# Ruyi-Zha/endosurf

Hardware: AMD Instinct MI355X
Metric: training rays/sec (1024 rays x 64 samples) (higher is better)
Workload: dtype f32

## Files before the change

### endosurf_amd/_lib.py

```python
from __future__ import annotations

import ctypes as C
import os

HERE = os.path.dirname(os.path.abspath(__file__))
LIB_PATH = os.path.join(HERE, "lib", "libendosurf_hip.so")

_c_float_p = C.c_void_p


class es_points(C.Structure):
    _fields_ = [("x", C.c_void_p), ("t", C.c_void_p), ("dirs", C.c_void_p), ("rays", C.c_void_p), ("z", C.c_void_p),
                ("mode", C.c_int), ("t_scalar", C.c_int), ("n_per_ray", C.c_int), ("ldz", C.c_int), ("M", C.c_int), ("M_split", C.c_int)]


class es_composite_args(C.Structure):
    _fields_ = ([(n, C.c_void_p) for n in ("rays", "z")] + [("ldz", C.c_int)]
                + [(n, C.c_void_p) for n in ("sdf", "g_o", "rgb", "variance")]
                + [("N", C.c_int), ("S", C.c_int), ("sample_dist", C.c_float), ("cos_anneal", C.c_float)]
                + [(n, C.c_void_p) for n in ("color", "depth", "weights", "cdf", "weight_max", "eik_acc", "wmax_idx",
                                             "g_color", "g_depth", "g_weights", "g_cdf", "g_wmax", "g_gradients_o", "g_eik",
                                             "eik_den", "d_sdf", "d_go", "d_rgb", "d_invs_acc", "ray_part", "cos_anneal_dev",
                                             "go_copy", "g_aux_sdf", "g_aux_go")] + [("n_aux", C.c_int)])

# ... 42 lines not shown
    "es_secant_points": (_I, [_P, _P, _I, _P, _P, _P]),
    "es_secant_update": (_I, [_P, _I, _F, _P, _P, _P]),
    "es_march_finish": (_I, [_P, _P, _I, _P, _P]),
    "es_point_workspace_floats": (C.c_int64, [_I, _I]),
    "es_point_workspace_offset": (C.c_int64, [_I, _I, _I]),
    "es_point_forward": (_I, [C.POINTER(es_points), _P, _P, _P, _I, _I, _P]),
    "es_point_forward_rows": (_I, [C.POINTER(es_points), _P, _P, _P, _I, _I, _I, _I, _P]),
    "es_eod_points": (_I, [_P, _P, _P, _I, _P, _P, _P, _P]),
    "es_sn_points": (_I, [_P, _P, _P, _P, _F, _I, _P, _P, _P, _P]),
    "es_eod_loss": (_I, [_P, _P, _P, _P, _P, _I, _P, _P, _P]),
    "es_eod_loss_backward": (_I, [_P, _P, _P, _P, _P, _P, _P, _I, _P, _P, _P]),
    "es_sn_loss": (_I, [_P, _P, _I, _P, _P]),
    "es_sn_loss_backward": (_I, [_P, _P, _P, _P, _I, _P, _P]),
    "es_copy2": (_I, [_P, _P, C.c_longlong, _P, _P, C.c_longlong, _P]),
    "es_color_forward": (_I, [C.POINTER(es_points), _P, _P, _P, _P]),
    "es_point_vjp": (_I, [C.POINTER(es_points), _P, _P, _P, _I, _P]),
    "es_point_backward_stages": (_I, [C.POINTER(es_points), _P, _P, _P, _I, _I, _P, _P, _P, _P, _P, _I, _P]),
    "es_weightnorm_backward_layers": (_I, [_P, _P, _P, _I, _I, _P]),
    "es_point_forward_x3": (_I, [C.POINTER(es_points), _P, _P, _P, _P, _I, _I, _P]),
    "es_gemm_atb": (_I, [_P, _P, _I, _P, _I, _P, _P]),
    "es_point_backward_x3": (_I, [C.POINTER(es_points), _P, _P, _P, _P, _I, _I, _P, _P, _P, _P, _P, _P]),
    "es_point_backward": (_I, [C.POINTER(es_points), _P, _P, _P, _I, _I, _P, _P, _P, _P, _P]),
    "es_wgrad_scratch_floats": (C.c_int64, []),
    "es_point_backward_det": (_I, [C.POINTER(es_points), _P, _P, _P, _I, _I, _P, _P, _P, _P, _P, _P]),
    "es_train_loss": (_I, [C.POINTER(es_loss_args), _P]),
    "es_query_sdf_rays": (_I, [C.POINTER(es_points), _P, _P, _P, _I, _P, _I, _P]),
    "es_march_progress": (_I, [_P, _I, _I, _I, C.c_float, _P, _P]),
    "es_variance_terms": (_I, [_P, _P, _P, _P, _P]),
    "es_sample_scratch_floats": (C.c_int64, [_I, _I, _I, _I]),
    "es_sample_z": (_I, [_P, _P, _I, _I, _I, _I, _I, _P, _P, _I, _P, _P, _P]),
    "es_march_scratch_floats": (C.c_int64, [_I, _I]),
    "es_ray_marching": (_I, [_P, _I, _I, _I, C.c_float, _I, _P, _P, _I, _P, _P, _P]),
    "es_render_scratch_floats": (C.c_int64, [_I, _I]),
    "es_render_forward": (_I, [C.POINTER(es_render_args), _P, _P, _P]),
    "es_render_backward": (_I, [C.POINTER(es_render_args), _P, _P, _P, _P]),
    "es_train_aux_points": (_I, [_P, _P, _P, _P, _P, C.c_float, _I, _P, _P, _P, _P]),
    "es_adam_step": (_I, [_P, _P, _P, _P, C.c_longlong, C.c_float, C.c_float, C.c_float, C.c_float, C.c_float, C.c_float, _P, C.c_longlong, _P]),
    "es_train_schedule": (_I, [_P, C.c_double, C.c_double, C.c_double, C.c_double, C.c_double, C.c_double, C.c_float, C.c_double, _P, _P]),
    "es_adam_step_dev": (_I, [_P, _P, _P, _P, C.c_longlong, C.c_float, C.c_float, C.c_float, _P, _P, C.c_longlong, _P]),
    "es_zero": (_I, [_P, C.c_longlong, _P]),
    "es_uniform": (_I, [_P, C.c_longlong, C.c_ulonglong, C.c_ulonglong, _P, _P]),
    "es_scale": (_I, [_P, _P, C.c_longlong, _P, _P]),
    "es_render_finish": (_I, [_P, _P, _P, _I, _P, _P, _P, _P, _P]),
    "es_iso_scratch_bytes": (C.c_int64, [_I, _I, _I]),
    "es_iso_count": (_I, [_P, _I, _I, _I, C.c_double, _P, _P, _P]),
    "es_iso_emit": (_I, [_P, _I, _I, _I, C.c_double, _P, C.c_longlong, C.c_longlong, _P, _P, _P, _P]),
# ... 105 lines not shown
```

### endosurf_amd/csrc/api.hip

```cpp
#include "arch.h"
#include "chain_common.h"
#include "host.h"
#include "launch.h"
#include "workspace.h"

namespace es {
static inline PointSrc to_src(const es_points* p) { PointSrc s; static_cast<es_points&>(s) = *p; return s; }
static inline int check_src(const es_points* p) {
    ES_REQUIRE(p != nullptr, "es_points is null");
    ES_REQUIRE(p->M >= 0, "negative point count");
    if (p->M == 0) return ST_OK;
    if (p->mode == 0) {
        ES_REQUIRE(p->x && p->t, "mode 0 needs x and t");
    } else {
        ES_REQUIRE(p->mode == 1 || p->mode == 2, "unknown point-source mode");
        ES_REQUIRE(p->rays && p->z && p->n_per_ray > 0 && p->ldz >= p->n_per_ray, "modes 1/2 need rays, z, n_per_ray <= ldz");
        if (p->mode == 2) ES_REQUIRE(p->M_split >= 0 && p->M_split <= p->M && (p->M_split == p->M || (p->x && p->t)), "mode 2 needs M_split <= M and x, t");
    }
    return ST_OK;
}
static inline int check_points(const es_points* p, bool weights, bool rows) {
    if (int e = check_src(p)) return e;
    ES_REQUIRE(weights && (rows || p->M == 0), "null buffer");
    return ST_OK;
// ... 246 lines not shown
int es_point_backward_x3(const es_points* pts, const float* packed, const void* packed_x3, const float* weff, float* ws, int flags, int m_color,
                         const float* d_sdf, const float* d_go, const float* d_rgb, float* dweff, float* wg_scratch, void* stream) {
    if (int e = check_point_call(pts, packed && packed_x3 && weff && dweff, ws && d_sdf && d_go, flags, m_color, true, d_rgb)) return e;
    flags |= ES_PF_X3_CHAIN | ES_PF_X3;
    return run_backward(pts, packed, packed_x3, weff, ws, flags, m_color, d_sdf, d_go, d_rgb, dweff, wg_scratch, 15, stream);
}
int es_point_backward_det(const es_points* pts, const float* packed, const float* weff, float* ws, int flags, int m_color,
                          const float* d_sdf, const float* d_go, const float* d_rgb, float* dweff, float* wg_scratch, void* stream) {
    if (int e = check_point_call(pts, packed && weff && dweff, ws && d_sdf && d_go, flags, m_color, true, d_rgb)) return e;
    return run_backward(pts, packed, nullptr, weff, ws, flags, m_color, d_sdf, d_go, d_rgb, dweff, wg_scratch, 15, stream);
}
int es_point_backward(const es_points* pts, const float* packed, const float* weff, float* ws, int flags, int m_color,
                      const float* d_sdf, const float* d_go, const float* d_rgb, float* dweff, void* stream) {
    return es_point_backward_det(pts, packed, weff, ws, flags, m_color, d_sdf, d_go, d_rgb, dweff, nullptr, stream);
}
int es_point_backward_stages(const es_points* pts, const float* packed, const float* weff, float* ws, int flags, int m_color,
                             const float* d_sdf, const float* d_go, const float* d_rgb, float* dweff, float* wg_scratch, int stages, void* stream) {
    if (int e = check_point_call(pts, packed && weff && dweff, ws && d_sdf && d_go, flags, m_color, true, d_rgb)) return e;
    ES_REQUIRE(!(flags & ES_PF_X3_CHAIN), "the staged backward is the fp32 family's (a workspace of es_point_forward)");
    ES_REQUIRE(stages > 0 && stages < 16, "stages: ES_BWD_CHAINS | ES_BWD_WGRAD_DEFORM | ES_BWD_WGRAD_SDF | ES_BWD_WGRAD_COLOR");
    return run_backward(pts, packed, nullptr, weff, ws, flags, m_color, d_sdf, d_go, d_rgb, dweff, wg_scratch, stages, stream);
}
int64_t es_wgrad_scratch_floats(void) { return (int64_t)wgrad_det_floats(); }
int es_gemm_atb(const float* X, const float* dA, int M, float* out, int split_precision, float* wg_scratch, void* stream) {
    ES_REQUIRE(X && dA && out && M > 0 && M % 64 == 0, "es_gemm_atb: X [M][256], dA [M][256], out [256][256], M a multiple of 64");
    return gemm_atb(X, dA, M, out, split_precision, wg_scratch, (hipStream_t)stream);
}

int es_train_loss(const es_loss_args* a, void* stream) {
    ES_REQUIRE(a && a->eik, "es_train_loss inputs");
    ES_REQUIRE(a->N == 0 || (a->color_map && a->depth_map && a->aux_sdf && a->aux_go && a->rays && a->eod_pts && a->color_gt && a->depth_gt &&
                             a->mask && a->cmask && a->valid_sn), "es_train_loss inputs");
    ES_REQUIRE(a->den_out || (a->terms && a->g_eik && (a->N == 0 || (a->g_color && a->g_depth && a->g_aux_sdf && a->g_aux_go))),
               "es_train_loss outputs");
    ES_REQUIRE(!a->den_global || a->world >= 1.f, "es_train_loss: den_global needs the world size");
    return train_loss(*reinterpret_cast<const LossArgs*>(a), (hipStream_t)stream);
}

int es_zero(void* p, long long nbytes, void* stream) {
    ES_REQUIRE((p || nbytes == 0) && nbytes >= 0, "es_zero arguments");
    return zero(p, nbytes, (hipStream_t)stream);
}
int es_uniform(float* out, long long n, unsigned long long seed, unsigned long long subsequence, const double* subsequence_dev, void* stream) {
    ES_REQUIRE((out || n == 0) && n >= 0, "es_uniform arguments");
    return uniform(out, n, seed, subsequence, subsequence_dev, (hipStream_t)stream);
}
// ... 38 lines not shown
```

### endosurf_amd/csrc/host.h

```cpp
#pragma once
#include <hip/hip_runtime.h>

#include <cstddef>
#include <type_traits>

#include "../../include/endosurf_hip.h"

namespace es {

struct PointSrc; struct WsLayout; struct FwdArgs; struct BwdArgs;

struct CompositeArgs : ::es_composite_args {};
struct LossArgs : ::es_loss_args {};
static_assert(sizeof(CompositeArgs) == sizeof(es_composite_args) && std::is_standard_layout<CompositeArgs>::value, "es::CompositeArgs is es_composite_args");
static_assert(sizeof(LossArgs) == sizeof(es_loss_args) && std::is_standard_layout<LossArgs>::value, "es::LossArgs is es_loss_args");
inline const CompositeArgs& as_comp(const es_composite_args* a) { return *reinterpret_cast<const CompositeArgs*>(a); }

int init_tables();
int weightnorm_pack(const float* params, float* weff, float* packed, int use_deform, hipStream_t st);
int weightnorm_backward(const float* params, const float* dweff, float* dparams, int use_deform, hipStream_t st);
int weightnorm_backward_layers(const float* params, const float* dweff, float* dparams, int first_layer, int n_layers, hipStream_t st);

int query_sdf(const PointSrc& src, const float* packed, const float* weff, float* sdf_out, int use_deform, hipStream_t st,
              int ld_out = 0, const int* ray_done = nullptr, int tile_points = 0);
// ... 3 lines not shown
int query_sdf_x3(const PointSrc& src, const void* packed_x3, const float* weff, float* sdf_out, int use_deform, hipStream_t st, int ld_out, const int* ray_done);

int point_forward(const PointSrc& src, const float* packed, const float* weff, float* ws, int flags, int m_color, hipStream_t st,
                  const void* packed_x3 = nullptr);
int point_forward_rows(const PointSrc& src, const float* packed, const float* weff, float* ws, int flags, int m_color, int row0, int nrows, hipStream_t st);
int point_vjp(const PointSrc& src, const float* packed, const float* weff, float* ws, int flags, hipStream_t st);
int color_forward(const PointSrc& src, const float* packed, const float* weff, float* ws, hipStream_t st);
int point_backward_chains(const PointSrc& src, const float* packed, const float* weff, float* ws, int flags, int m_color,
                          const float* d_sdf, const float* d_go, const float* d_rgb, hipStream_t st, const void* packed_x3 = nullptr);

int deform_jvp_x3r(const PointSrc& src, const void* packed_r, const float* weff, float* ws, const WsLayout& L, bool save, hipStream_t st);
int deform_vjp_x3r(const PointSrc& src, const void* packed_r, const float* weff, float* ws, const WsLayout& L, bool save, hipStream_t st, int m_rows = 0);
int deform_jvp_x3r_with_tail(const FwdArgs& fa, const void* packed_r, int m_main, hipStream_t st);
int sdf_fwd_x3r(const PointSrc& src, const void* packed_r, const float* weff, float* ws, const WsLayout& L, bool deform, bool color, hipStream_t st);
int color_fwd_x3r(const PointSrc& src, const void* packed_r, const float* weff, float* ws, const WsLayout& L, bool deform, int Mcp, bool save, hipStream_t st);

int deform_tan_x3r(const PointSrc& src, const void* packed_r, const float* weff, float* ws, const WsLayout& L, const float* d_go, hipStream_t st, int m_rows = 0);
int deform_bwd_x3r_with_tail(const BwdArgs& ba, const void* packed_r, int m_main, hipStream_t st);
int color_bwd_x3r(const PointSrc& src, const void* packed_r, const float* weff, float* ws, const WsLayout& L, bool deform, int m_color, const float* d_rgb, hipStream_t st);
int deform_bwd_x3r(const void* packed_r, const float* weff, float* ws, const WsLayout& L, int M, int m_color, hipStream_t st);

int point_wgrad(int M, float* ws, int flags, int m_color, const float* d_sdf, float* dweff, float* det, hipStream_t st, int net_mask = 7);
size_t wgrad_det_floats();
int gemm_atb(const float* X, const float* dA, int M, float* out, int x3, float* det, hipStream_t st);

int ray_setup(const float* rays, const float* u, int N, int n, float sample_dist, int lin_mode, float* z, int ldz, float* near_out, float* far_out, hipStream_t st);
int upsample_step(const float* rays, const float* z_in, int ld_in, const float* sdf_in, int ld_sdf, int N, int n, int n_imp,
                  float inv_s, float* z_new, float* z_out, int ld_out, int* src_idx, hipStream_t st);
int merge_sdf(const float* sdf_in, int ld_in, const float* sdf_new, int n_imp, const int* src_idx, int ld_out, int N, int n, float* sdf_out, hipStream_t st);
int mid_z(const float* z, int ldz, int N, int S, float sample_dist, float* mid, hipStream_t st);
int composite(const CompositeArgs& a, int backward, hipStream_t st);
int variance_terms(const float* variance, const float* d_invs_acc, float* s_val, float* d_var, hipStream_t st);
int march_progress(const float* sdf, int N, int n, int n_valid, float tau, int* done, hipStream_t st);
int march_find(const float* sdf, const float* dprop, int N, int n, float tau, float* state, int* flags, float* d_pred, hipStream_t st);
int secant_points(const float* rays, const float* d_pred, int N, float* x, float* t, hipStream_t st);
int secant_update(const float* sdf_mid, int N, float tau, float* state, float* d_pred, hipStream_t st);
int march_finish(const float* d_pred, const int* flags, int N, float* d_out, hipStream_t st);
int train_aux_points(const float* rays, const float* depth_gt, const float* mask, const float* d_i, const float* u, float rad, int N, float* x, float* t, unsigned char* valid, hipStream_t st);

int eod_points(const float* rays, const float* depth_gt, const float* mask, int N, float* x, float* t, float* inside, hipStream_t st);
int sn_points(const float* rays, const float* mask, const float* d_i, const float* u, float rad, int N, float* x, float* t, unsigned char* valid, hipStream_t st);
int eod_loss(const float* rays, const float* pts, const float* mask, const float* sdf, const float* go, int N, float* out, float* inside, hipStream_t st);
int eod_loss_bwd(const float* rays, const float* inside, const float* sdf, const float* go, const float* out, const float* g_sdf_err,
                 const float* g_ang_err, int N, float* d_sdf, float* d_go, hipStream_t st);
int sn_loss(const float* g, const unsigned char* valid, int N, float* out, hipStream_t st);
int sn_loss_bwd(const float* g, const unsigned char* valid, const float* out, const float* g_loss, int N, float* d_g, hipStream_t st);
// ... 14 lines not shown
```

### endosurf_amd/csrc/wgrad.hip

```cpp
#include <hip/hip_runtime.h>

#include <type_traits>
#include <utility>

#include "arch.h"
#include "chain_common.h"
#include "host.h"
#include "launch.h"
#include "tabs.h"
#include "timing.h"
#include "workspace.h"

namespace es {

constexpr int WG_MAX_PROBS = 20;

struct WgProb {
    const float* X; const float* dA; float* out; float* bias_out;
    int ldx, lda, ldo, M, K, N, bias_stride, task_begin;
    int x_frag, a_frag;
    int round;
};
struct WgSmall {
    const float* X; const float* dA; float* out; float* bias_out;
    int ldx, lda, ldo, M, K, N, bias_stride, x_frag, round;
};
constexpr int WG_MAX_SMALL = 4;
constexpr int WG_MAX_TASKS = 512;
struct WgArgs {
    WgProb p[WG_MAX_PROBS];
    WgSmall s[WG_MAX_SMALL];
    int nprob, total_tasks, MC, nsmall;
    int KW;
    float* det;
};
constexpr size_t WG_DET_TILE = (size_t)256 * 128;
constexpr size_t WG_DET_BIAS_OFF = (size_t)WG_MAX_TASKS * WG_DET_TILE;
constexpr size_t WG_DET_SMALL_OFF = WG_DET_BIAS_OFF + (size_t)WG_MAX_TASKS * 256;
constexpr size_t WG_DET_FLOATS = WG_DET_SMALL_OFF + (size_t)WG_MAX_SMALL * WG_MAX_TASKS * 5 * 256;

__host__ __device__ inline void wg_decode(int local, int kblk, int nchunk, int& kb, int& mc) {
    if (kblk == 2) {
        const int grp = local / 16, j = local % 16;
        const int full = (nchunk / 8) * 8;
        if (grp * 8 < full) { mc = grp * 8 + (j & 7); kb = j >> 3; }
        else { const int rem = local - 2 * full; kb = rem & 1; mc = full + (rem >> 1); }
    } else { kb = local % kblk; mc = local / kblk; }
}
__host__ __device__ inline int wg_encode(int kb, int mc, int kblk, int nchunk) {
    if (kblk == 2) {
        const int full = (nchunk / 8) * 8;
        return mc < full ? (mc / 8) * 16 + (mc & 7) + 8 * kb : 2 * full + (((mc - full) << 1) | kb);
    }
    return mc * kblk + kb;
}

constexpr int WG_THREADS = 512;
constexpr int WG_R = 16;
constexpr int WG_KW = 128;
constexpr int WG_LDS_FLOATS = 2 * WG_R * (256 + WG_KW);

template <bool AF, bool XF, bool DET>
__device__ __forceinline__ void wgrad_task(const WgProb& P, int kb, int m0, int m1, float* lds, float* det_tile, float* det_bias) {
    constexpr int KW = WG_KW;
    const int tid = threadIdx.x, lane = tid & 63;
    const int w = __builtin_amdgcn_readfirstlane(tid >> 6);
    const int nb = w & 3, kh = w >> 2;
    const int lo = lane & 31, hi = lane >> 5;
    auto Apan = [&](int buf) { return lds + buf * (WG_R * 256); };
    auto Bpan = [&](int buf) { return lds + 2 * WG_R * 256 + buf * (WG_R * KW); };
    const int kcol0 = kb * KW;

    typedef float v4f_t __attribute__((ext_vector_type(4)));
    f32x16 acc[2][2];
    acc_zero(acc);
    const bool do_bias = P.bias_out != nullptr && kb == 0;
    v4f_t bsum = {0.f, 0.f, 0.f, 0.f};

    typedef float v4f __attribute__((ext_vector_type(4)));
    const v4f vzero = {0.f, 0.f, 0.f, 0.f};
    const int fa1 = tid + WG_THREADS;
    const unsigned offA0 = (unsigned)(tid >> 6) * (unsigned)P.lda + 4u * (tid & 63);
    const int colB = kcol0 + 4 * (tid % (KW / 4));
    const unsigned offB = (unsigned)(tid / (KW / 4)) * (unsigned)P.ldx + (unsigned)colB;
    const bool okB = XF || colB < P.ldx;
    const int fqq = (tid >> 6) & 1, fni = (tid >> 7) & 1, fw = tid >> 8;
    const unsigned foffA0 = (unsigned)(((fw * 16 + fni * 4 + fqq) * 64 + lane) * 4);
    const unsigned foffB = (unsigned)((((2 * kb + fw) * 16 + fni * 4 + fqq) * 64 + lane) * 4);
    const int flrow = 8 * fqq + 4 * hi;
    const int flcolA = 64 * fw + 32 * fni + lo, flcolB = 64 * fw + 32 * fni + lo;
    const unsigned boffA0 = 4u * (AF ? foffA0 : offA0), boffB = 4u * (XF ? foffB : offB);
    const size_t dA1 = AF ? (size_t)2 * 16 * 64 * 4 * 4 : (size_t)8 * P.lda * 4;
    auto stage_ptr = [&](const float* base, int ld, bool frag, int m) {
        return frag ? base + (size_t)(m >> 6) * (64 * 256) + (size_t)((8 * ((m >> 5) & 1) + 2 * ((m >> 4) & 1)) * 256) : base + (size_t)m * ld;
    };
#define WG_GLOAD(S, m)                                                                                \
    {                                                                                                 \
        const char* pa = reinterpret_cast<const char*>(stage_ptr(P.dA, P.lda, AF, m));                \
        unsigned oa0 = boffA0, ob = boffB;                                                            \
        asm volatile("" : "+v"(oa0), "+v"(ob));       \
        S##a0 = *reinterpret_cast<const v4f*>(pa + oa0);                                              \
        S##a1 = *reinterpret_cast<const v4f*>(pa + dA1 + oa0);       \
        const char* px = reinterpret_cast<const char*>(stage_ptr(P.X, P.ldx, XF, m));                 \
        S##b0 = okB ? *reinterpret_cast<const v4f*>(px + ob) : vzero;                                 \
    }
#define WG_SSTORE(S, buf)                                                                             \
    {                                                                                                 \
        if constexpr (AF) {                                                                           \
            float* la = Apan(buf) + flrow * 256 + flcolA;                                             \
            la[0] = S##a0[0]; la[256] = S##a0[1]; la[512] = S##a0[2]; la[768] = S##a0[3];             \
            la[128] = S##a1[0]; la[128 + 256] = S##a1[1]; la[128 + 512] = S##a1[2]; la[128 + 768] = S##a1[3]; \
            bsum[0] += S##a0[0] + S##a0[1] + S##a0[2] + S##a0[3];                                     \
            bsum[1] += S##a1[0] + S##a1[1] + S##a1[2] + S##a1[3];                                     \
        } else {                                                                                      \
            *reinterpret_cast<v4f*>(Apan(buf) + 4 * tid) = S##a0;                                     \
            *reinterpret_cast<v4f*>(Apan(buf) + 4 * fa1) = S##a1;                                     \
            bsum += S##a0 + S##a1;                                                                    \
        }                                                                                             \
        if constexpr (XF) {                                                                           \
            float* lb = Bpan(buf) + flrow * KW + flcolB;                                              \
            lb[0] = S##b0[0]; lb[KW] = S##b0[1]; lb[2 * KW] = S##b0[2]; lb[3 * KW] = S##b0[3];        \
        } else {                                                                                      \
            *reinterpret_cast<v4f*>(Bpan(buf) + 4 * tid) = S##b0;                                     \
        }                                                                                             \
    }
    auto compute = [&](int buf) {
        const float* A = Apan(buf) + nb * 64 + 2 * lo;
        const float* B = Bpan(buf) + kh * 64 + 2 * lo;
#pragma unroll
        for (int s = 0; s < WG_R / 2; ++s) {
            const float2 av = *reinterpret_cast<const float2*>(A + (2 * s + hi) * 256);
            const float2 bv = *reinterpret_cast<const float2*>(B + (2 * s + hi) * KW);
            acc[0][0] = __builtin_amdgcn_mfma_f32_32x32x2f32(av.x, bv.x, acc[0][0], 0, 0, 0);
            acc[0][1] = __builtin_amdgcn_mfma_f32_32x32x2f32(av.x, bv.y, acc[0][1], 0, 0, 0);
            acc[1][0] = __builtin_amdgcn_mfma_f32_32x32x2f32(av.y, bv.x, acc[1][0], 0, 0, 0);
            acc[1][1] = __builtin_amdgcn_mfma_f32_32x32x2f32(av.y, bv.y, acc[1][1], 0, 0, 0);
        }
    };

    const int nst = (m1 - m0) / WG_R;
    v4f p0a0, p0a1, p0b0, p1a0, p1a1, p1b0;
    WG_GLOAD(p0, m0);
    WG_GLOAD(p1, m0 + WG_R);
    WG_SSTORE(p0, 0);
    __syncthreads();
#pragma unroll 1
    for (int st = 0; st < nst; st += 2) {
        if (st + 2 < nst) WG_GLOAD(p0, m0 + WG_R * (st + 2));
        compute(0);
        WG_SSTORE(p1, 1);
        __syncthreads();
        if (st + 3 < nst) WG_GLOAD(p1, m0 + WG_R * (st + 3));
        compute(1);
        if (st + 2 < nst) WG_SSTORE(p0, 0);
        __syncthreads();
    }
#undef WG_GLOAD
#undef WG_SSTORE
    int tid_e = threadIdx.x;
    asm volatile("" : "+v"(tid_e));
    const int lane_e = tid_e & 63, lo_e = lane_e & 31, hi_e = lane_e >> 5;
#pragma unroll
    for (int t = 0; t < 2; ++t)
#pragma unroll
        for (int tp = 0; tp < 2; ++tp) {
            const int k = kcol0 + kh * 64 + 2 * lo_e + tp;
#pragma unroll
            for (int r = 0; r < 16; ++r) {
                const int n = nb * 64 + 2 * ((r & 3) + 8 * (r >> 2) + 4 * hi_e) + t;
                if constexpr (DET) det_tile[n * WG_KW + (k - kcol0)] = acc[t][tp][r];
                else if (n < P.N && k < P.K) atomicAdd(P.out + (size_t)n * P.ldo + k, acc[t][tp][r]);
            }
        }
    if (do_bias) {
        if (!AF && ((tid_e >> 6) & (P.bias_stride - 1)) != 0) bsum = v4f{0.f, 0.f, 0.f, 0.f};
        __syncthreads();
        if constexpr (AF) {
            const int fqq_e = (tid_e >> 6) & 1, col_e = 64 * (tid_e >> 8) + 32 * ((tid_e >> 7) & 1) + lo_e;
            lds[(fqq_e * 2 + hi_e) * 256 + col_e] = bsum[0];
            lds[(fqq_e * 2 + hi_e) * 256 + col_e + 128] = bsum[1];
        } else {
            *reinterpret_cast<v4f*>(lds + 4 * tid_e) = bsum;
        }
        __syncthreads();
        if (tid_e < 256) {
            float s = 0.f;
#pragma unroll
            for (int r = 0; r < (AF ? 4 : 8); ++r) s += lds[r * 256 + tid_e];
            if constexpr (DET) det_bias[tid_e] = s;
            else if (tid_e < P.N) atomicAdd(P.bias_out + tid_e, s);
        }
    }
}

constexpr int WS_ROWS = 16;
template <bool DET, int NH = 2>
// ... 57 lines not shown
    __syncthreads();
    float* red = lds;
    if (NH == 2 && half) {
#pragma unroll
        for (int n = 0; n < 4; ++n) red[n * 256 + k] = acc[n];
        red[1024 + k] = bsum;
    }
    if (NH == 2) __syncthreads();
    if (!half) {
        if constexpr (NH == 2) {
#pragma unroll
            for (int n = 0; n < 4; ++n) acc[n] += red[n * 256 + k];
            bsum += red[1024 + k];
        }
        if constexpr (DET) {
            for (int n = 0; n < 4; ++n) det_slot[n * 256 + k] = acc[n];
            det_slot[4 * 256 + k] = bsum;
        } else {
            for (int n = 0; n < P.N; ++n) atomicAdd(P.out + (size_t)n * P.ldo + k, acc[n]);
            if (P.bias_out && k < P.N) atomicAdd(P.bias_out + k, bsum);
        }
    }
    __syncthreads();
}

template <int NET, bool DET>
__global__ __launch_bounds__(WG_THREADS, 4) void k_wgrad(WgArgs a) {
    extern __shared__ __attribute__((aligned(16))) float wlds[];
    const int task = blockIdx.x;
    auto small_slot = [&](int i) { return DET ? a.det + WG_DET_SMALL_OFF + ((size_t)i * WG_MAX_TASKS + task) * (5 * 256) : nullptr; };
    const bool small_first = task < a.total_tasks / 2;
    if (small_first)
#pragma unroll 1
        for (int i = 0; i < a.nsmall; ++i) wgrad_small_task<DET>(a.s[i], task, a.total_tasks, wlds, small_slot(i));
    int pi = 0;
#pragma unroll 1
    for (int i = 1; i < a.nprob; ++i)
        if (task >= a.p[i].task_begin) pi = i;
    const WgProb& P = a.p[pi];
    const int local = task - P.task_begin;
    const int kblk = (P.K + WG_KW - 1) / WG_KW;
    int kb, mc;
    wg_decode(local, kblk, (P.M + a.MC - 1) / a.MC, kb, mc);
    const int m0 = mc * a.MC, m1 = min(m0 + a.MC, P.M);
    float* dt = DET ? a.det + (size_t)task * WG_DET_TILE : nullptr;
    float* db = DET ? a.det + WG_DET_BIAS_OFF + (size_t)task * 256 : nullptr;
    if constexpr (NET == 1) {
        if (P.a_frag) {
            if (P.x_frag) wgrad_task<true, true, DET>(P, kb, m0, m1, wlds, dt, db);
            else wgrad_task<true, false, DET>(P, kb, m0, m1, wlds, dt, db);
        } else {
            if (P.x_frag) wgrad_task<false, true, DET>(P, kb, m0, m1, wlds, dt, db);
            else wgrad_task<false, false, DET>(P, kb, m0, m1, wlds, dt, db);
        }
    } else {
        wgrad_task<false, false, DET>(P, kb, m0, m1, wlds, dt, db);
    }
    if (!small_first) {
        __syncthreads();
#pragma unroll 1
        for (int i = 0; i < a.nsmall; ++i) wgrad_small_task<DET>(a.s[i], task, a.total_tasks, wlds, small_slot(i));
    }
}


typedef unsigned wx_u32x4 __attribute__((ext_vector_type(4)));
typedef __bf16 wx_bf16x8 __attribute__((ext_vector_type(8)));
constexpr int WX_THREADS = 256;
constexpr int WX_R = 16;
constexpr int WX_KW = 256;
constexpr int WX_PLANE = 2 * 256 * 16;
constexpr int WX_BUF = 6 * WX_PLANE;
constexpr int WX_NBUF = 3;
constexpr int WX_LDS_BYTES = WX_NBUF * WX_BUF;
static_assert(WX_LDS_BYTES >= WG_LDS_FLOATS * 4, "the small-layer slices reuse the buffer as float scratch");

__device__ __forceinline__ unsigned wx_cvt_pk(float lo, float hi) {
    unsigned r;
    asm("v_cvt_pk_bf16_f32 %0, %1, %2" : "=v"(r) : "v"(lo), "v"(hi));
// ... 209 lines not shown
    if constexpr (NET == 1) {
        if (P.a_frag) {
            if (P.x_frag) wgrad_task_x3<true, true, DET>(P, m0, m1, wxlds, dt, db);
            else wgrad_task_x3<true, false, DET>(P, m0, m1, wxlds, dt, db);
        } else {
            if (P.x_frag) wgrad_task_x3<false, true, DET>(P, m0, m1, wxlds, dt, db);
            else wgrad_task_x3<false, false, DET>(P, m0, m1, wxlds, dt, db);
        }
    } else {
        wgrad_task_x3<false, false, DET>(P, m0, m1, wxlds, dt, db);
    }
    if (!small_first) {
#pragma unroll 1
        for (int i = 0; i < a.nsmall; ++i) wgrad_small_task<DET, 1>(a.s[i], task, a.total_tasks, wlds, small_slot(i));
    }
}

__global__ __launch_bounds__(256) void k_wgrad_reduce(WgArgs a, int round) {
    const int pi = blockIdx.y;
    const int tid0 = blockIdx.x * 256 + threadIdx.x, stride = gridDim.x * 256;
    if (pi < a.nprob) {
        const WgProb& P = a.p[pi];
        if (P.round != round) return;
        const int kblk = (P.K + a.KW - 1) / a.KW, nchunk = (P.M + a.MC - 1) / a.MC;
        const size_t tile = (size_t)256 * a.KW;
        for (int e = tid0; e < P.N * P.K; e += stride) {
            const int n = e / P.K, k = e % P.K, kb = k / a.KW, kk = k % a.KW;
            float s = 0.f;
            for (int mc = 0; mc < nchunk; ++mc)
                s += a.det[(size_t)(P.task_begin + wg_encode(kb, mc, kblk, nchunk)) * tile + n * a.KW + kk];
            P.out[(size_t)n * P.ldo + k] += s;
        }
        if (P.bias_out)
            for (int n = tid0; n < P.N; n += stride) {
                float s = 0.f;
                for (int mc = 0; mc < nchunk; ++mc)
                    s += a.det[WG_DET_BIAS_OFF + (size_t)(P.task_begin + wg_encode(0, mc, kblk, nchunk)) * 256 + n];
                P.bias_out[n] += s;
            }
    } else {
        const int i = pi - a.nprob;
        const WgSmall& P = a.s[i];
        if (P.round != round) return;
        const float* base = a.det + WG_DET_SMALL_OFF + (size_t)i * WG_MAX_TASKS * (5 * 256);
        for (int e = tid0; e < P.N * 256; e += stride) {
            const int n = e >> 8, k = e & 255;
            float s = 0.f;
            for (int t = 0; t < a.total_tasks; ++t) s += base[(size_t)t * (5 * 256) + n * 256 + k];
            P.out[(size_t)n * P.ldo + k] += s;
        }
        if (P.bias_out)
            for (int n = tid0; n < P.N; n += stride) {
                float s = 0.f;
                for (int t = 0; t < a.total_tasks; ++t) s += base[(size_t)t * (5 * 256) + 4 * 256 + n];
                P.bias_out[n] += s;
            }
    }
}

static int wg_kblk(const WgProb& p, int kw) { return (p.K + kw - 1) / kw; }

static int launch_group(WgProb* probs, int nprob, WgSmall* small, int nsmall, int kid_timer, long long rows, float* det, bool x3, hipStream_t st) {
    const int kid = kid_timer == KID_WGRAD_D_X3 ? KID_WGRAD_D : (kid_timer == KID_WGRAD_S_X3 ? KID_WGRAD_S : (kid_timer == KID_WGRAD_C_X3 ? KID_WGRAD_C : kid_timer));
    static DeviceOnce attr_done;
    if (attr_done.first()) {
        if (int e = allow_big_lds(k_wgrad<0, false>, WG_LDS_FLOATS * 4)) return e;
        if (int e = allow_big_lds(k_wgrad<1, false>, WG_LDS_FLOATS * 4)) return e;
        if (int e = allow_big_lds(k_wgrad<2, false>, WG_LDS_FLOATS * 4)) return e;
        if (int e = allow_big_lds(k_wgrad<0, true>, WG_LDS_FLOATS * 4)) return e;
        if (int e = allow_big_lds(k_wgrad<1, true>, WG_LDS_FLOATS * 4)) return e;
        if (int e = allow_big_lds(k_wgrad<2, true>, WG_LDS_FLOATS * 4)) return e;
        if (int e = allow_big_lds(k_wgrad_x3<0, false>, WX_LDS_BYTES)) return e;
        if (int e = allow_big_lds(k_wgrad_x3<1, false>, WX_LDS_BYTES)) return e;
        if (int e = allow_big_lds(k_wgrad_x3<2, false>, WX_LDS_BYTES)) return e;
        if (int e = allow_big_lds(k_wgrad_x3<0, true>, WX_LDS_BYTES)) return e;
        if (int e = allow_big_lds(k_wgrad_x3<1, true>, WX_LDS_BYTES)) return e;
        if (int e = allow_big_lds(k_wgrad_x3<2, true>, WX_LDS_BYTES)) return e;
        attr_done.done();
    }
    if (nprob == 0) return ST_OK;
    ES_REQUIRE(nprob <= WG_MAX_PROBS, "too many weight-gradient problems in one group");
    const int KW = x3 ? WX_KW : WG_KW;
    auto count = [&](int mc) {
        long long t = 0;
        for (int i = 0; i < nprob; ++i) t += (long long)wg_kblk(probs[i], KW) * ((probs[i].M + mc - 1) / mc);
        return t;
    };
    ES_REQUIRE(nsmall <= WG_MAX_SMALL, "too many small weight-gradient problems in one group");
    int MC = 128;
    const int slots = x3 ? WG_MAX_TASKS / 2 : WG_MAX_TASKS;
    while (MC < 65536 && count(MC) > slots) MC += 64;
    ES_REQUIRE(count(MC) <= slots, "weight-gradient group does not fit one round of workgroup slots");
    WgArgs a;
    a.det = det;
    int total = 0, max_round = 0;
    for (int i = 0; i < nprob; ++i) {
        ES_REQUIRE(probs[i].lda == 256 && probs[i].M % 64 == 0, "weight-gradient operands must be [64k][256] adjoints");
        ES_REQUIRE((probs[i].bias_stride & (probs[i].bias_stride - 1)) == 0, "bias stride must be a power of two");
        ES_REQUIRE(!probs[i].a_frag || probs[i].bias_stride == 1 || !probs[i].bias_out, "fragment-ordered adjoints: bias over every row");
        ES_REQUIRE(!probs[i].x_frag || (probs[i].ldx == 256 && probs[i].K == 256), "fragment-ordered inputs are [64 x 256] tiles");
        ES_REQUIRE(kid == KID_WGRAD_S || !(probs[i].x_frag || probs[i].a_frag), "fragment-ordered operands: SDF launch only");
        probs[i].task_begin = total;
        total += wg_kblk(probs[i], KW) * ((probs[i].M + MC - 1) / MC);
        probs[i].round = 0;
        for (int j = 0; j < i; ++j)
            if (probs[j].out == probs[i].out && probs[j].round >= probs[i].round) probs[i].round = probs[j].round + 1;
        max_round = probs[i].round > max_round ? probs[i].round : max_round;
        a.p[i] = probs[i];
    }
    a.nprob = nprob; a.total_tasks = total; a.MC = MC; a.nsmall = nsmall; a.KW = KW;
    for (int i = 0; i < nsmall; ++i) {
        ES_REQUIRE(small[i].K == 256 && small[i].N <= 4, "small weight-gradient problems are [<=4 x 256]");
        small[i].round = 0;
        for (int j = 0; j < i; ++j)
            if (small[j].out == small[i].out && small[j].round >= small[i].round) small[i].round = small[j].round + 1;
        max_round = small[i].round > max_round ? small[i].round : max_round;
        a.s[i] = small[i];
    }
    const dim3 grid(total);
    ScopedTimer tm(kid_timer, rows, st);
    if (x3) {
        auto reduce = [&]() {
            for (int r = 0; det && r <= max_round; ++r)
                hipLaunchKernelGGL(k_wgrad_reduce, dim3(32, nprob + nsmall), dim3(256), 0, st, a, r);
        };
        if (det) {
// ... 114 lines not shown
```

### include/endosurf_hip.h

```cpp
#ifndef ENDOSURF_HIP_H
#define ENDOSURF_HIP_H

#include <stddef.h>
#include <stdint.h>

#ifdef __cplusplus
extern "C" {
#endif

#define ES_ABI_VERSION 14

int es_abi_version(void);
const char* es_last_error(void);
int es_init(void);

int64_t es_param_floats(void);
int es_param_layout(int net, int layer, int64_t* bias_off, int64_t* g_off, int64_t* v_off, int* out_dim, int* in_dim);
int64_t es_param_variance_off(void);
int64_t es_weff_floats(void);
int es_weff_layout(int net, int layer, int64_t* w_off, int64_t* b_off);
int64_t es_packed_floats(void);

int es_weightnorm_pack(const float* params, float* weff, float* packed, int use_deform, void* stream);
int es_weightnorm_backward(const float* params, const float* dweff, float* dparams, int use_deform, void* stream);
// ... 87 lines not shown
int es_point_forward_rows(const es_points* pts, const float* packed, const float* weff, float* ws, int flags, int m_color, int row0, int nrows,
                          void* stream);
int es_point_vjp(const es_points* pts, const float* packed, const float* weff, float* ws, int flags, void* stream);
int es_color_forward(const es_points* pts, const float* packed, const float* weff, float* ws, void* stream);
int es_point_forward_x3(const es_points* pts, const float* packed, const void* packed_x3, const float* weff, float* ws, int flags, int m_color,
                        void* stream);
int es_gemm_atb(const float* X, const float* dA, int M, float* out, int split_precision, float* wg_scratch, void* stream);
int es_point_backward_x3(const es_points* pts, const float* packed, const void* packed_x3, const float* weff, float* ws, int flags, int m_color,
                         const float* d_sdf, const float* d_go, const float* d_rgb, float* dweff, float* wg_scratch, void* stream);
int es_point_backward(const es_points* pts, const float* packed, const float* weff, float* ws, int flags, int m_color,
                      const float* d_sdf, const float* d_go, const float* d_rgb, float* dweff, void* stream);

#define ES_BWD_CHAINS 1
#define ES_BWD_WGRAD_DEFORM 2
#define ES_BWD_WGRAD_SDF 4
#define ES_BWD_WGRAD_COLOR 8
int es_point_backward_stages(const es_points* pts, const float* packed, const float* weff, float* ws, int flags, int m_color,
                             const float* d_sdf, const float* d_go, const float* d_rgb, float* dweff, float* wg_scratch, int stages, void* stream);

int64_t es_wgrad_scratch_floats(void);
int es_point_backward_det(const es_points* pts, const float* packed, const float* weff, float* ws, int flags, int m_color,
                          const float* d_sdf, const float* d_go, const float* d_rgb, float* dweff, float* wg_scratch, void* stream);

int es_timing_enable(int on);
int es_timing_drain(int capacity, int* kid, long long* rows, float* ms, int* n_out);
const char* es_kernel_name(int kid);

typedef struct es_loss_args {
    const float* color_map; const float* depth_map; const float* eik; const float* aux_sdf; const float* aux_go;
    const float* rays; const float* eod_pts; const float* color_gt; const float* depth_gt; const float* mask; const float* cmask;
    const unsigned char* valid_sn;
    int N;
    float w_color, w_depth, w_sdf, w_angle, w_eik, w_sn;
    float* terms; float* g_color; float* g_depth; float* g_eik; float* g_aux_sdf; float* g_aux_go;
    float* den_out; const float* den_global; float world;
    float* total_out;
} es_loss_args;
int es_train_loss(const es_loss_args* a, void* stream);

int es_train_aux_points(const float* rays, const float* depth_gt, const float* mask, const float* d_i, const float* u, float rad, int N,
                        float* x, float* t, unsigned char* valid, void* stream);

int es_eod_points(const float* rays, const float* depth_gt, const float* mask, int N, float* x, float* t, float* inside, void* stream);
int es_sn_points(const float* rays, const float* mask, const float* d_i, const float* u, float rad, int N, float* x, float* t,
                 unsigned char* valid, void* stream);
int es_eod_loss(const float* rays, const float* pts, const float* mask, const float* sdf, const float* g_o, int N, float* out, float* inside,
// ... 102 lines not shown
```

Before: 72960.

## Specialize weight-gradient tasks by live column width and balance chunk rows per class

Adds width classes for weight-gradient k-blocks that are only partly live (at most 64 or at most 96 columns). For these, the dead half-tile skips its MFMA work or uses a single-column MFMA path, and dead B loads are replaced with zeros. A new planner gives each problem its own chunk row count, weighted by per-class cost, so narrow problems take longer M chunks and the tasks in one launch round are balanced. The cost is more template instantiations and a heuristic cost table that may not match the hardware.

```diff
diff --git a/endosurf_amd/_lib.py b/endosurf_amd/_lib.py
--- a/endosurf_amd/_lib.py
+++ b/endosurf_amd/_lib.py
@@ -88,6 +88,8 @@
     "es_point_backward_x3": (_I, [C.POINTER(es_points), _P, _P, _P, _P, _I, _I, _P, _P, _P, _P, _P, _P]),
     "es_point_backward": (_I, [C.POINTER(es_points), _P, _P, _P, _I, _I, _P, _P, _P, _P, _P]),
     "es_wgrad_scratch_floats": (C.c_int64, []),
+    "es_wgrad_plan": (_I, [_P, _P, _I, _I, _P, _P]),
+    "es_wgrad_width_cost": (C.c_double, [_I]),
     "es_point_backward_det": (_I, [C.POINTER(es_points), _P, _P, _P, _I, _I, _P, _P, _P, _P, _P, _P]),
     "es_train_loss": (_I, [C.POINTER(es_loss_args), _P]),
     "es_query_sdf_rays": (_I, [C.POINTER(es_points), _P, _P, _P, _I, _P, _I, _P]),
diff --git a/endosurf_amd/csrc/api.hip b/endosurf_amd/csrc/api.hip
--- a/endosurf_amd/csrc/api.hip
+++ b/endosurf_amd/csrc/api.hip
@@ -292,6 +292,10 @@
     return run_backward(pts, packed, nullptr, weff, ws, flags, m_color, d_sdf, d_go, d_rgb, dweff, wg_scratch, stages, stream);
 }
 int64_t es_wgrad_scratch_floats(void) { return (int64_t)wgrad_det_floats(); }
+int es_wgrad_plan(const int* rows, const int* cols, int nprob, int slots, int* chunk_rows, int* chunks) {
+    return wgrad_plan(rows, cols, nprob, slots, chunk_rows, chunks);
+}
+double es_wgrad_width_cost(int cols) { return wgrad_width_cost(cols); }
 int es_gemm_atb(const float* X, const float* dA, int M, float* out, int split_precision, float* wg_scratch, void* stream) {
     ES_REQUIRE(X && dA && out && M > 0 && M % 64 == 0, "es_gemm_atb: X [M][256], dA [M][256], out [256][256], M a multiple of 64");
     return gemm_atb(X, dA, M, out, split_precision, wg_scratch, (hipStream_t)stream);
diff --git a/endosurf_amd/csrc/host.h b/endosurf_amd/csrc/host.h
--- a/endosurf_amd/csrc/host.h
+++ b/endosurf_amd/csrc/host.h
@@ -49,6 +49,8 @@
 
 int point_wgrad(int M, float* ws, int flags, int m_color, const float* d_sdf, float* dweff, float* det, hipStream_t st, int net_mask = 7);
 size_t wgrad_det_floats();
+int wgrad_plan(const int* rows, const int* cols, int nprob, int slots, int* chunk_rows, int* chunks);
+double wgrad_width_cost(int cols);
 int gemm_atb(const float* X, const float* dA, int M, float* out, int x3, float* det, hipStream_t st);
 
 int ray_setup(const float* rays, const float* u, int N, int n, float sample_dist, int lin_mode, float* z, int ldz, float* near_out, float* far_out, hipStream_t st);
diff --git a/endosurf_amd/csrc/wgrad.hip b/endosurf_amd/csrc/wgrad.hip
--- a/endosurf_amd/csrc/wgrad.hip
+++ b/endosurf_amd/csrc/wgrad.hip
@@ -20,6 +20,7 @@
     int ldx, lda, ldo, M, K, N, bias_stride, task_begin;
     int x_frag, a_frag;
     int round;
+    int MC, nchunk;
 };
 struct WgSmall {
     const float* X; const float* dA; float* out; float* bias_out;
@@ -54,14 +55,19 @@
     }
     return mc * kblk + kb;
 }
+__host__ __device__ inline int wg_width_class(int K, int kb) {
+    const int live = K - kb * 128;
+    return live <= 64 ? 1 : (live <= 96 ? 2 : 0);
+}
 
 constexpr int WG_THREADS = 512;
 constexpr int WG_R = 16;
 constexpr int WG_KW = 128;
 constexpr int WG_LDS_FLOATS = 2 * WG_R * (256 + WG_KW);
 
-template <bool AF, bool XF, bool DET>
+template <bool AF, bool XF, bool DET, int WC>
 __device__ __forceinline__ void wgrad_task(const WgProb& P, int kb, int m0, int m1, float* lds, float* det_tile, float* det_bias) {
+    static_assert(!XF || WC == 0, "fragment-ordered inputs are 256 columns wide: every k-block is full");
     constexpr int KW = WG_KW;
     const int tid = threadIdx.x, lane = tid & 63;
     const int w = __builtin_amdgcn_readfirstlane(tid >> 6);
@@ -89,7 +95,8 @@
     const unsigned foffB = (unsigned)((((2 * kb + fw) * 16 + fni * 4 + fqq) * 64 + lane) * 4);
     const int flrow = 8 * fqq + 4 * hi;
     const int flcolA = 64 * fw + 32 * fni + lo, flcolB = 64 * fw + 32 * fni + lo;
-    const unsigned boffA0 = 4u * (AF ? foffA0 : offA0), boffB = 4u * (XF ? foffB : offB);
+    const bool deadB = WC != 0 && !okB;
+    const unsigned boffA0 = 4u * (AF ? foffA0 : offA0), boffB = 4u * (XF ? foffB : (deadB ? 0u : offB));
     const size_t dA1 = AF ? (size_t)2 * 16 * 64 * 4 * 4 : (size_t)8 * P.lda * 4;
     auto stage_ptr = [&](const float* base, int ld, bool frag, int m) {
         return frag ? base + (size_t)(m >> 6) * (64 * 256) + (size_t)((8 * ((m >> 5) & 1) + 2 * ((m >> 4) & 1)) * 256) : base + (size_t)m * ld;
@@ -102,7 +109,8 @@
         S##a0 = *reinterpret_cast<const v4f*>(pa + oa0);                                              \
         S##a1 = *reinterpret_cast<const v4f*>(pa + dA1 + oa0);       \
         const char* px = reinterpret_cast<const char*>(stage_ptr(P.X, P.ldx, XF, m));                 \
-        S##b0 = okB ? *reinterpret_cast<const v4f*>(px + ob) : vzero;                                 \
+        if constexpr (WC != 0) S##b0 = *reinterpret_cast<const v4f*>(px + ob);                        \
+        else S##b0 = okB ? *reinterpret_cast<const v4f*>(px + ob) : vzero;                            \
     }
 #define WG_SSTORE(S, buf)                                                                             \
     {                                                                                                 \
@@ -121,20 +129,36 @@
             float* lb = Bpan(buf) + flrow * KW + flcolB;                                              \
             lb[0] = S##b0[0]; lb[KW] = S##b0[1]; lb[2 * KW] = S##b0[2]; lb[3 * KW] = S##b0[3];        \
         } else {                                                                                      \
-            *reinterpret_cast<v4f*>(Bpan(buf) + 4 * tid) = S##b0;                                     \
+            *reinterpret_cast<v4f*>(Bpan(buf) + 4 * tid) = deadB ? vzero : S##b0;                     \
         }                                                                                             \
     }
-    auto compute = [&](int buf) {
-        const float* A = Apan(buf) + nb * 64 + 2 * lo;
-        const float* B = Bpan(buf) + kh * 64 + 2 * lo;
-#pragma unroll
-        for (int s = 0; s < WG_R / 2; ++s) {
-            const float2 av = *reinterpret_cast<const float2*>(A + (2 * s + hi) * 256);
-            const float2 bv = *reinterpret_cast<const float2*>(B + (2 * s + hi) * KW);
-            acc[0][0] = __builtin_amdgcn_mfma_f32_32x32x2f32(av.x, bv.x, acc[0][0], 0, 0, 0);
-            acc[0][1] = __builtin_amdgcn_mfma_f32_32x32x2f32(av.x, bv.y, acc[0][1], 0, 0, 0);
-            acc[1][0] = __builtin_amdgcn_mfma_f32_32x32x2f32(av.y, bv.x, acc[1][0], 0, 0, 0);
-            acc[1][1] = __builtin_amdgcn_mfma_f32_32x32x2f32(av.y, bv.y, acc[1][1], 0, 0, 0);
+    f32x16 acc1[2];
+#pragma unroll
+    for (int r = 0; r < 16; ++r) acc1[0][r] = acc1[1][r] = 0.f;
+    auto compute = [&](int buf, auto mode_c) {
+        constexpr int MODE = decltype(mode_c)::value;
+        if constexpr (MODE == 0) {
+            const float* A = Apan(buf) + nb * 64 + 2 * lo;
+            const float* B = Bpan(buf) + kh * 64 + 2 * lo;
+#pragma unroll
+            for (int s = 0; s < WG_R / 2; ++s) {
+                const float2 av = *reinterpret_cast<const float2*>(A + (2 * s + hi) * 256);
+                const float2 bv = *reinterpret_cast<const float2*>(B + (2 * s + hi) * KW);
+                acc[0][0] = __builtin_amdgcn_mfma_f32_32x32x2f32(av.x, bv.x, acc[0][0], 0, 0, 0);
+                acc[0][1] = __builtin_amdgcn_mfma_f32_32x32x2f32(av.x, bv.y, acc[0][1], 0, 0, 0);
+                acc[1][0] = __builtin_amdgcn_mfma_f32_32x32x2f32(av.y, bv.x, acc[1][0], 0, 0, 0);
+                acc[1][1] = __builtin_amdgcn_mfma_f32_32x32x2f32(av.y, bv.y, acc[1][1], 0, 0, 0);
+            }
+        } else if constexpr (MODE == 2) {
+            const float* A = Apan(buf) + nb * 64 + 2 * lo;
+            const float* B = Bpan(buf) + kh * 64 + lo;
+#pragma unroll
+            for (int s = 0; s < WG_R / 2; ++s) {
+                const float2 av = *reinterpret_cast<const float2*>(A + (2 * s + hi) * 256);
+                const float bv = B[(2 * s + hi) * KW];
+                acc1[0] = __builtin_amdgcn_mfma_f32_32x32x2f32(av.x, bv, acc1[0], 0, 0, 0);
+                acc1[1] = __builtin_amdgcn_mfma_f32_32x32x2f32(av.y, bv, acc1[1], 0, 0, 0);
+            }
         }
     };
 
@@ -144,34 +168,47 @@
     WG_GLOAD(p1, m0 + WG_R);
     WG_SSTORE(p0, 0);
     __syncthreads();
-#pragma unroll 1
-    for (int st = 0; st < nst; st += 2) {
-        if (st + 2 < nst) WG_GLOAD(p0, m0 + WG_R * (st + 2));
-        compute(0);
-        WG_SSTORE(p1, 1);
-        __syncthreads();
-        if (st + 3 < nst) WG_GLOAD(p1, m0 + WG_R * (st + 3));
-        compute(1);
-        if (st + 2 < nst) WG_SSTORE(p0, 0);
-        __syncthreads();
-    }
+#define WG_STAGE_LOOP(MODE)                                                                           \
+    _Pragma("unroll 1") for (int st = 0; st < nst; st += 2) {                                         \
+        if (st + 2 < nst) WG_GLOAD(p0, m0 + WG_R * (st + 2));                                         \
+        compute(0, std::integral_constant<int, MODE>());                                              \
+        WG_SSTORE(p1, 1);                                  \
+        __syncthreads();                                                                              \
+        if (st + 3 < nst) WG_GLOAD(p1, m0 + WG_R * (st + 3));                                         \
+        compute(1, std::integral_constant<int, MODE>());                                              \
+        if (st + 2 < nst) WG_SSTORE(p0, 0);                                           \
+        __syncthreads();                                                                              \
+    }
+    if constexpr (WC == 0) {
+        WG_STAGE_LOOP(0)
+    } else if (kh == 0) {
+        WG_STAGE_LOOP(0)
+    } else {
+        WG_STAGE_LOOP(WC)
+        if constexpr (WC == 2) { acc[0][0] = acc1[0]; acc[1][0] = acc1[1]; }
+    }
+#undef WG_STAGE_LOOP
 #undef WG_GLOAD
 #undef WG_SSTORE
     int tid_e = threadIdx.x;
     asm volatile("" : "+v"(tid_e));
     const int lane_e = tid_e & 63, lo_e = lane_e & 31, hi_e = lane_e >> 5;
-#pragma unroll
-    for (int t = 0; t < 2; ++t)
-#pragma unroll
-        for (int tp = 0; tp < 2; ++tp) {
-            const int k = kcol0 + kh * 64 + 2 * lo_e + tp;
-#pragma unroll
-            for (int r = 0; r < 16; ++r) {
-                const int n = nb * 64 + 2 * ((r & 3) + 8 * (r >> 2) + 4 * hi_e) + t;
-                if constexpr (DET) det_tile[n * WG_KW + (k - kcol0)] = acc[t][tp][r];
-                else if (n < P.N && k < P.K) atomicAdd(P.out + (size_t)n * P.ldo + k, acc[t][tp][r]);
-            }
-        }
+    const bool one_tile = WC == 2 && kh == 1;
+    if (WC != 1 || kh == 0) {
+#pragma unroll
+        for (int t = 0; t < 2; ++t)
+#pragma unroll
+            for (int tp = 0; tp < 2; ++tp) {
+                if (one_tile && tp == 1) continue;
+                const int k = kcol0 + kh * 64 + (one_tile ? lo_e : 2 * lo_e + tp);
+#pragma unroll
+                for (int r = 0; r < 16; ++r) {
+                    const int n = nb * 64 + 2 * ((r & 3) + 8 * (r >> 2) + 4 * hi_e) + t;
+                    if constexpr (DET) det_tile[n * WG_KW + (k - kcol0)] = acc[t][tp][r];
+                    else if (n < P.N && k < P.K) atomicAdd(P.out + (size_t)n * P.ldo + k, acc[t][tp][r]);
+                }
+            }
+    }
     if (do_bias) {
         if (!AF && ((tid_e >> 6) & (P.bias_stride - 1)) != 0) bsum = v4f{0.f, 0.f, 0.f, 0.f};
         __syncthreads();
@@ -275,6 +312,18 @@
         }
     }
     __syncthreads();
+}
+
+template <bool AF, bool XF, bool DET>
+__device__ __forceinline__ void wgrad_task_wc(const WgProb& P, int kb, int m0, int m1, float* lds, float* det_tile, float* det_bias) {
+    if constexpr (XF) {
+        wgrad_task<AF, true, DET, 0>(P, kb, m0, m1, lds, det_tile, det_bias);
+    } else {
+        const int wc = wg_width_class(P.K, kb);
+        if (wc == 1) wgrad_task<AF, false, DET, 1>(P, kb, m0, m1, lds, det_tile, det_bias);
+        else if (wc == 2) wgrad_task<AF, false, DET, 2>(P, kb, m0, m1, lds, det_tile, det_bias);
+        else wgrad_task<AF, false, DET, 0>(P, kb, m0, m1, lds, det_tile, det_bias);
+    }
 }
 
 template <int NET, bool DET>
@@ -294,20 +343,20 @@
     const int local = task - P.task_begin;
     const int kblk = (P.K + WG_KW - 1) / WG_KW;
     int kb, mc;
-    wg_decode(local, kblk, (P.M + a.MC - 1) / a.MC, kb, mc);
-    const int m0 = mc * a.MC, m1 = min(m0 + a.MC, P.M);
+    wg_decode(local, kblk, P.nchunk, kb, mc);
+    const int m0 = mc * P.MC, m1 = min(m0 + P.MC, P.M);
     float* dt = DET ? a.det + (size_t)task * WG_DET_TILE : nullptr;
     float* db = DET ? a.det + WG_DET_BIAS_OFF + (size_t)task * 256 : nullptr;
     if constexpr (NET == 1) {
         if (P.a_frag) {
-            if (P.x_frag) wgrad_task<true, true, DET>(P, kb, m0, m1, wlds, dt, db);
-            else wgrad_task<true, false, DET>(P, kb, m0, m1, wlds, dt, db);
+            if (P.x_frag) wgrad_task_wc<true, true, DET>(P, kb, m0, m1, wlds, dt, db);
+            else wgrad_task_wc<true, false, DET>(P, kb, m0, m1, wlds, dt, db);
         } else {
-            if (P.x_frag) wgrad_task<false, true, DET>(P, kb, m0, m1, wlds, dt, db);
-            else wgrad_task<false, false, DET>(P, kb, m0, m1, wlds, dt, db);
+            if (P.x_frag) wgrad_task_wc<false, true, DET>(P, kb, m0, m1, wlds, dt, db);
+            else wgrad_task_wc<false, false, DET>(P, kb, m0, m1, wlds, dt, db);
         }
     } else {
-        wgrad_task<false, false, DET>(P, kb, m0, m1, wlds, dt, db);
+        wgrad_task_wc<false, false, DET>(P, kb, m0, m1, wlds, dt, db);
     }
     if (!small_first) {
         __syncthreads();
@@ -563,7 +612,7 @@
     if (pi < a.nprob) {
         const WgProb& P = a.p[pi];
         if (P.round != round) return;
-        const int kblk = (P.K + a.KW - 1) / a.KW, nchunk = (P.M + a.MC - 1) / a.MC;
+        const int kblk = (P.K + a.KW - 1) / a.KW, nchunk = P.nchunk;
         const size_t tile = (size_t)256 * a.KW;
         for (int e = tid0; e < P.N * P.K; e += stride) {
             const int n = e / P.K, k = e % P.K, kb = k / a.KW, kk = k % a.KW;
@@ -600,6 +649,68 @@
 }
 
 static int wg_kblk(const WgProb& p, int kw) { return (p.K + kw - 1) / kw; }
+
+constexpr double WG_CLASS_COST[3] = {1.0, 0.60, 0.82};
+static_assert(WG_CLASS_COST[0] >= WG_CLASS_COST[2] && WG_CLASS_COST[2] >= WG_CLASS_COST[1], "wgrad_plan walks the costliest class present");
+double wgrad_width_cost(int cols) { return WG_CLASS_COST[cols > 128 ? 0 : wg_width_class(cols, 0)]; }
+
+int wgrad_plan(const int* rows, const int* cols, int nprob, int slots, int* chunk_rows, int* chunks) {
+    ES_REQUIRE(rows && cols && chunk_rows && chunks && nprob > 0 && nprob <= WG_MAX_PROBS && slots > 0, "wgrad_plan: 1 .. 20 problems, slots > 0");
+    int cls[WG_MAX_PROBS], kblk[WG_MAX_PROBS], max_rows = 0;
+    bool present[3] = {false, false, false};
+    for (int i = 0; i < nprob; ++i) {
+        ES_REQUIRE(rows[i] > 0 && rows[i] % 64 == 0 && cols[i] > 0, "wgrad_plan: rows a positive multiple of 64, cols > 0");
+        kblk[i] = (cols[i] + WG_KW - 1) / WG_KW;
+        cls[i] = kblk[i] > 1 ? 0 : wg_width_class(cols[i], 0);
+        present[cls[i]] = true;
+        max_rows = rows[i] > max_rows ? rows[i] : max_rows;
+    }
+    auto count = [&](const int (&L)[3]) {
+        long long t = 0;
+        for (int i = 0; i < nprob; ++i) t += (long long)kblk[i] * ((rows[i] + L[cls[i]] - 1) / L[cls[i]]);
+        return t;
+    };
+    auto slot_time = [&](const int (&L)[3]) {
+        double s = 0.0;
+        for (int c = 0; c < 3; ++c)
+            if (present[c] && L[c] * WG_CLASS_COST[c] > s) s = L[c] * WG_CLASS_COST[c];
+        return s;
+    };
+    int best[3] = {128, 128, 128};
+    bool found = count(best) <= slots;
+    const int base = present[0] ? 0 : (present[2] ? 2 : 1);
+    int other[2], nother = 0;
+    for (int c = 1; c < 3; ++c)
+        if (present[c] && c != base) other[nother++] = c;
+    for (int Lb = 128; !found && Lb < max_rows + 64; Lb += 64) {
+        double best_time = 0.0;
+        long long best_tasks = 0;
+        for (int combo = 0; combo < (1 << nother); ++combo) {
+            int L[3] = {Lb, Lb, Lb};
+            for (int j = 0; j < nother; ++j) {
+                const int below = (int)(Lb * WG_CLASS_COST[base] / WG_CLASS_COST[other[j]]) / 64 * 64;
+                L[other[j]] = (below < 128 ? 128 : below) + 64 * ((combo >> j) & 1);
+            }
+            const long long tasks = count(L);
+            if (tasks > slots) continue;
+            const double t = slot_time(L);
+            if (!found || t < best_time || (t == best_time && tasks < best_tasks)) {
+                found = true; best_time = t; best_tasks = tasks;
+                for (int c = 0; c < 3; ++c) best[c] = L[c];
+            }
+        }
+    }
+    ES_REQUIRE(found, "weight-gradient group does not fit one round of workgroup slots");
+    int one[3] = {128, 128, 128};
+    while (count(one) > slots) one[0] = one[1] = one[2] = one[0] + 64;
+    if (slot_time(one) <= slot_time(best))
+        for (int c = 0; c < 3; ++c) best[c] = one[c];
+    for (int i = 0; i < nprob; ++i) {
+        chunk_rows[i] = best[cls[i]] < rows[i] ? best[cls[i]] : rows[i];
+        chunks[i] = (rows[i] + chunk_rows[i] - 1) / chunk_rows[i];
+    }
+    return ST_OK;
+}
 
 static int launch_group(WgProb* probs, int nprob, WgSmall* small, int nsmall, int kid_timer, long long rows, float* det, bool x3, hipStream_t st) {
     const int kid = kid_timer == KID_WGRAD_D_X3 ? KID_WGRAD_D : (kid_timer == KID_WGRAD_S_X3 ? KID_WGRAD_S : (kid_timer == KID_WGRAD_C_X3 ? KID_WGRAD_C : kid_timer));
@@ -629,9 +740,18 @@
     };
     ES_REQUIRE(nsmall <= WG_MAX_SMALL, "too many small weight-gradient problems in one group");
     int MC = 128;
-    const int slots = x3 ? WG_MAX_TASKS / 2 : WG_MAX_TASKS;
-    while (MC < 65536 && count(MC) > slots) MC += 64;
-    ES_REQUIRE(count(MC) <= slots, "weight-gradient group does not fit one round of workgroup slots");
+    for (int i = 0; i < nprob; ++i) ES_REQUIRE(probs[i].M > 0 && probs[i].M % 64 == 0, "weight-gradient operands must be [64k][256] adjoints");
+    if (x3) {
+        const int slots = WG_MAX_TASKS / 2;
+        while (MC < 65536 && count(MC) > slots) MC += 64;
+        ES_REQUIRE(count(MC) <= slots, "weight-gradient group does not fit one round of workgroup slots");
+        for (int i = 0; i < nprob; ++i) { probs[i].MC = MC; probs[i].nchunk = (probs[i].M + MC - 1) / MC; }
+    } else {
+        int rows[WG_MAX_PROBS], cols[WG_MAX_PROBS], chunk_rows[WG_MAX_PROBS], chunks[WG_MAX_PROBS];
+        for (int i = 0; i < nprob; ++i) { rows[i] = probs[i].M; cols[i] = probs[i].K; }
+        if (int e = wgrad_plan(rows, cols, nprob, WG_MAX_TASKS, chunk_rows, chunks)) return e;
+        for (int i = 0; i < nprob; ++i) { probs[i].MC = chunk_rows[i]; probs[i].nchunk = chunks[i]; }
+    }
     WgArgs a;
     a.det = det;
     int total = 0, max_round = 0;
@@ -642,7 +762,7 @@
         ES_REQUIRE(!probs[i].x_frag || (probs[i].ldx == 256 && probs[i].K == 256), "fragment-ordered inputs are [64 x 256] tiles");
         ES_REQUIRE(kid == KID_WGRAD_S || !(probs[i].x_frag || probs[i].a_frag), "fragment-ordered operands: SDF launch only");
         probs[i].task_begin = total;
-        total += wg_kblk(probs[i], KW) * ((probs[i].M + MC - 1) / MC);
+        total += wg_kblk(probs[i], KW) * probs[i].nchunk;
         probs[i].round = 0;
         for (int j = 0; j < i; ++j)
             if (probs[j].out == probs[i].out && probs[j].round >= probs[i].round) probs[i].round = probs[j].round + 1;
diff --git a/include/endosurf_hip.h b/include/endosurf_hip.h
--- a/include/endosurf_hip.h
+++ b/include/endosurf_hip.h
@@ -133,6 +133,9 @@
 int es_point_backward_det(const es_points* pts, const float* packed, const float* weff, float* ws, int flags, int m_color,
                           const float* d_sdf, const float* d_go, const float* d_rgb, float* dweff, float* wg_scratch, void* stream);
 
+int es_wgrad_plan(const int* rows, const int* cols, int nprob, int slots, int* chunk_rows, int* chunks);
+double es_wgrad_width_cost(int cols);
+
 int es_timing_enable(int on);
 int es_timing_drain(int capacity, int* kid, long long* rows, float* ms, int* n_out);
 const char* es_kernel_name(int kid);
```

After: 72860. No clear change (-0.1%).
